# NVlabs/FoundationPose

Measured on NVIDIA H100. Metric: pose-hypotheses/sec at 640x480 RGB-D, 252 hyp, 5 refine iters, higher is better.
Workload: dtype f16

## Files before the change

### foundationpose_b200/csrc/fp_api_ops.cu

```cuda
#include "../../include/fpose.h"
#include "fp_common.cuh"
#include "fp_attn.cuh"
#include "fp_crop.cuh"
#include "fp_gemm.cuh"

#include <vector>

namespace fp {
const char* get_last_error();
int prof_collect(int kind, double* total_ms, double* total_work, int* launches);
int pose_errors_launch(const float* pts, int P, const float* pred, int N, const float* gt, int n_gt, float* add_out,
                       float* adds_out, cudaStream_t stream);
}

static int check_device_ptr(const void* p, const char* what) {
  int dev = 0;
  FP_CUDA_OK(cudaGetDevice(&dev));
  cudaPointerAttributes a;
  const cudaError_t e = cudaPointerGetAttributes(&a, p);
  if (e != cudaSuccess) {
    cudaGetLastError();
    fp::set_last_error("fp_pose_errors: %s: cudaPointerGetAttributes failed (%s)", what, cudaGetErrorString(e));
    return -1;
  }
// ... 97 lines not shown
  ap.k_off = 512;
  ap.v_off = 1024;
  ap.group_col_stride = 0;
  ap.n_groups = 1;
  ap.out = reinterpret_cast<__half*>(out);
  ap.ld_out = 512;
  ap.out_group_stride = 0;
  ap.B = B;
  ap.T = 400;
  ap.n_heads = 4;
  ap.scale = 0.08838834764831845f;
  cudaStream_t st = reinterpret_cast<cudaStream_t>(stream);
  (void)impl;
  return fp::attn_tc_launch(ap, st);
}

static fp::GemmLayer to_gemm_layer(const fp_gemm_layer_t* l) {
  fp::GemmLayer L;
  L.kind = l->kind;
  L.n_img = l->n_img;
  L.Hin = l->Hin;
  L.Win = l->Win;
  L.Cin = l->Cin;
  L.Cout = l->Cout;
  L.in = l->in;
  L.w = l->w;
  L.bias = l->bias;
  L.res = l->res;
  L.res_ld = l->res_ld;
  L.out = l->out;
  L.out_ld = l->out_ld;
  L.out_split = l->out_split;
  L.post_add = l->post_add;
  L.relu = l->relu;
  return L;
}

int fp_op_gemm_layer(const fp_gemm_layer_t* l, void* stream) {
  if (!l) {
    fp::set_last_error("fp_op_gemm_layer: null layer");
    return -1;
  }
  return fp::gemm_layer_launch(to_gemm_layer(l), reinterpret_cast<cudaStream_t>(stream));
}

int fp_op_gemm_tile_n(const fp_gemm_layer_t* l, int* tile_n) {
  if (!l || !tile_n) {
    fp::set_last_error("fp_op_gemm_tile_n: null argument");
    return -1;
  }
  return fp::gemm_layer_tile_n(to_gemm_layer(l), tile_n);
}

int fp_pose_errors(const float* pts, int P, const float* pred, int N, const float* gt, int n_gt, float* add_out,
                   float* adds_out, void* stream) {
  FP_REQUIRE(P >= 1 && P <= FP_METRICS_MAX_POINTS, "fp_pose_errors: P = %d outside [1, %d]", P, FP_METRICS_MAX_POINTS);
  FP_REQUIRE(N >= 0 && N <= FP_METRICS_MAX_POSES, "fp_pose_errors: N = %d outside [0, %d]", N, FP_METRICS_MAX_POSES);
  FP_REQUIRE(n_gt == 1 || n_gt == N, "fp_pose_errors: n_gt = %d, must be 1 or N = %d", n_gt, N);
  if (N == 0) return 0;
  FP_REQUIRE(pts && pred && gt, "fp_pose_errors: null input pointer");
  const void* ptrs[5] = {pts, pred, gt, add_out, adds_out};
  const char* names[5] = {"pts", "pred", "gt", "add_out", "adds_out"};
  for (int i = 0; i < 5; ++i)
    if (ptrs[i] && check_device_ptr(ptrs[i], names[i])) return -1;
  return fp::pose_errors_launch(pts, P, pred, N, gt, n_gt, add_out, adds_out, reinterpret_cast<cudaStream_t>(stream));
}

}
```

### foundationpose_b200/csrc/fp_common.cuh

```cuda
#pragma once
#include <cuda.h>
#include <cuda_fp16.h>
#include <cuda_runtime.h>
#include <stdint.h>
#include <stdio.h>
#include <string.h>

#include <atomic>

namespace fp {

void note_launches(int n);
unsigned long long launch_count();
void set_capturing(bool on);
inline bool device_bit_test(const std::atomic<unsigned long long>& m) {
  int d = 0;
  cudaGetDevice(&d);
  return (m.load(std::memory_order_acquire) >> (d & 63)) & 1ull;
}
inline void device_bit_set(std::atomic<unsigned long long>& m) {
  int d = 0;
  cudaGetDevice(&d);
  m.fetch_or(1ull << (d & 63), std::memory_order_release);
}
// ... 104 lines not shown
  asm volatile("cp.async.bulk.tensor.5d.global.shared::cta.bulk_group [%0, {%2, %3, %4, %5, %6}], [%1];" ::"l"(
                   reinterpret_cast<uint64_t>(map)),
               "r"(smem_u32(src)), "r"(c0), "r"(c1), "r"(c2), "r"(c3), "r"(c4)
               : "memory");
}
__device__ __forceinline__ void tma_prefetch_desc(const CUtensorMap* map) {
  asm volatile("prefetch.tensormap [%0];" ::"l"(reinterpret_cast<uint64_t>(map)) : "memory");
}

__device__ __forceinline__ uint32_t cluster_nctarank() {
  uint32_t r;
  asm volatile("mov.u32 %0, %%cluster_nctarank;" : "=r"(r));
  return r;
}
__device__ __forceinline__ uint32_t cluster_ctarank() {
  uint32_t r;
  asm volatile("mov.u32 %0, %%cluster_ctarank;" : "=r"(r));
  return r;
}
__device__ __forceinline__ void cluster_sync_all() {
  asm volatile("barrier.cluster.arrive.release.aligned;" ::: "memory");
  asm volatile("barrier.cluster.wait.acquire.aligned;" ::: "memory");
}

template <uint32_t N>
__device__ __forceinline__ void regs_release() {
  asm volatile("setmaxnreg.dec.sync.aligned.u32 %0;" ::"n"(N));
}
template <uint32_t N>
__device__ __forceinline__ void regs_acquire() {
  asm volatile("setmaxnreg.inc.sync.aligned.u32 %0;" ::"n"(N));
}

__device__ __forceinline__ void wgmma_fence() { asm volatile("wgmma.fence.sync.aligned;" ::: "memory"); }
__device__ __forceinline__ void wgmma_commit() { asm volatile("wgmma.commit_group.sync.aligned;" ::: "memory"); }
template <int N>
__device__ __forceinline__ void wgmma_wait() {
  asm volatile("wgmma.wait_group.sync.aligned %0;" ::"n"(N) : "memory");
}
template <int N>
__device__ __forceinline__ void fence_regs(float (&d)[N]) {
#pragma unroll
  for (int i = 0; i < N; ++i) asm volatile("" : "+f"(d[i])::"memory");
}

__device__ __forceinline__ uint64_t gmma_desc_sw128(uint32_t smem_addr, uint32_t sbo = 1024) {
  uint64_t d = 0;
  d |= (uint64_t)((smem_addr & 0x3FFFF) >> 4);
  d |= (uint64_t)1 << 16;
  d |= (uint64_t)(sbo >> 4) << 32;
  d |= (uint64_t)1 << 62;
  return d;
}
__device__ __forceinline__ uint64_t gmma_desc_mn_sw128(uint32_t smem_addr, uint32_t lbo) {
  uint64_t d = 0;
  d |= (uint64_t)((smem_addr & 0x3FFFF) >> 4);
  d |= (uint64_t)((lbo >> 4) & 0x3FFF) << 16;
  d |= (uint64_t)(1024 >> 4) << 32;
  d |= (uint64_t)1 << 62;
  return d;
}
__device__ __forceinline__ uint64_t gmma_desc_linear(uint32_t smem_addr, uint32_t lbo, uint32_t sbo) {
  uint64_t d = 0;
  d |= (uint64_t)((smem_addr & 0x3FFFF) >> 4);
  d |= (uint64_t)(lbo >> 4) << 16;
  d |= (uint64_t)(sbo >> 4) << 32;
  return d;
}

__device__ __forceinline__ uint32_t pack_half2(float a, float b) {
  __half2 h = __floats2half2_rn(a, b);
  return *reinterpret_cast<uint32_t*>(&h);
}

}
```

### foundationpose_b200/csrc/fp_gemm.cu

```cuda
#include "fp_gemm.cuh"

#include <stdarg.h>
#include <stdlib.h>
#include <string.h>

#include <mutex>
#include <vector>

#include "fp_common.cuh"
#include "fp_wgmma.cuh"

namespace fp {

static std::atomic<unsigned long long> g_launch_count{0};
static thread_local bool t_capturing = false;
void note_launches(int n) {
  if (!t_capturing) g_launch_count.fetch_add((unsigned long long)n, std::memory_order_relaxed);
}
unsigned long long launch_count() { return g_launch_count.load(std::memory_order_relaxed); }
void set_capturing(bool on) { t_capturing = on; }

std::atomic<bool> g_prof_on{false};
static std::mutex g_prof_mu;

// ... 49 lines not shown

static thread_local char t_last_error[1024] = "";
void set_last_error(const char* fmt, ...) {
  va_list ap;
  va_start(ap, fmt);
  vsnprintf(t_last_error, sizeof(t_last_error), fmt, ap);
  va_end(ap);
}
const char* get_last_error() { return t_last_error; }

static thread_local int t_pdl_skip = 0;
void pdl_skip_next() { t_pdl_skip = 1; }

bool pdl_enabled() {
  if (t_pdl_skip) {
    t_pdl_skip = 0;
    return false;
  }
  static int on = -1;
  if (on < 0) {
    const char* e = getenv("FPOSE_PDL");
    on = (e && e[0] == '0') ? 0 : 1;
  }
  return on != 0;
}

struct GemmParams {
  int lg_bw, lg_bh;
  int bw, bh, bn;
  int tiles_w, tiles_h, tiles_n, n_tiles_n, total_tiles;
  int num_kb, chunks_per_tap;
  int dim_w, dim_h, dim_n;
  short tap_off[9][5];
  int Ho, Wo, n_img, Cout;
  const float* bias;
  int has_res;
  int odim_h, odim_n;
  int out_split;
  const float* post_add;
  int relu;
  double alg_flops;
};

constexpr int kBlockM = 128;
constexpr int kBlockK = 64;
constexpr int kABytes = kBlockM * kBlockK * 2;
constexpr int kTileThreads = 384;
constexpr int kSlabBytes = kBlockM * 64 * 2;
constexpr int kSmemOptIn = 232448;

constexpr int kWideSlabs = 2;
constexpr int kWideProducerRegs = 40;
constexpr int kWideConsumerRegs = 232;
template <int BN>
struct TileCfg {
  static constexpr int kBBytes = BN * kBlockK * 2;
  static constexpr int kStageBytes = kABytes + kBBytes;
  static constexpr int kBatches = BN / 64;
  static constexpr bool kAlternate = BN > 128;
  static constexpr int kSlabs = kAlternate ? kWideSlabs : kBatches;
  static constexpr int kStagingBytes = kSlabs * kSlabBytes;
  static constexpr int kRing = kSmemOptIn - kStagingBytes - 1024  - 256 ;
  static constexpr int kStages = (kRing / kStageBytes) > 8 ? 8 : (kRing / kStageBytes);
  static constexpr int kSmemBytes = kStages * kStageBytes + kStagingBytes + 1024 + 256;
  static_assert(kSmemBytes <= kSmemOptIn, "tile configuration exceeds the 227 KB opt-in shared memory");
  static_assert((2 * kStages + kSlabs) * 8 <= 256, "the mbarriers must fit their 256 bytes");
  static_assert(kBatches % kSlabs == 0, "every slab must take the same number of batches per tile");
};

template <int BN>
__global__ void __launch_bounds__(kTileThreads, 1)
    gemm_tile_kernel(const __grid_constant__ CUtensorMap map_a, const __grid_constant__ CUtensorMap map_b,
                     const __grid_constant__ CUtensorMap map_out, const __grid_constant__ CUtensorMap map_res,
                     const __grid_constant__ GemmParams p) {
  using Cfg = TileCfg<BN>;
  constexpr int S = Cfg::kStages;
  constexpr int NSLAB = Cfg::kSlabs;
  constexpr int NB = Cfg::kBatches;
  constexpr bool kAlt = Cfg::kAlternate;
  extern __shared__ uint8_t smem_raw[];
  uint8_t* smem = smem_raw + ((1024u - (smem_u32(smem_raw) & 1023u)) & 1023u);
  uint8_t* staging = smem + S * Cfg::kStageBytes;
  uint64_t* bars = reinterpret_cast<uint64_t*>(staging + Cfg::kStagingBytes);
  uint64_t* full = bars;
  uint64_t* empty = bars + S;
  uint64_t* res_full = bars + 2 * S;

  const int m_tiles = p.tiles_w * p.tiles_h * p.tiles_n;
  const int total = m_tiles * p.n_tiles_n;

  if (threadIdx.x == 0) {
    tma_prefetch_desc(&map_a);
    tma_prefetch_desc(&map_b);
    tma_prefetch_desc(&map_out);
    if (p.has_res) tma_prefetch_desc(&map_res);
    for (int s = 0; s < S; ++s) {
      mbar_init(&full[s], 1);
      mbar_init(&empty[s], 256);
    }
    for (int s = 0; s < (kAlt ? NSLAB : 1); ++s) mbar_init(&res_full[s], 1);
    mbar_fence_init();
  }
  __syncthreads();
  pdl_trigger();
  pdl_wait();

  auto decode = [&](int t, int& n_tile, int& tw, int& th, int& tn) {
    n_tile = t % p.n_tiles_n;
    const int m_tile = t / p.n_tiles_n;
    tw = m_tile % p.tiles_w;
    th = (m_tile / p.tiles_w) % p.tiles_h;
    tn = m_tile / (p.tiles_w * p.tiles_h);
  };

  if (threadIdx.x < 128) {
    if constexpr (BN > 128) regs_release<kWideProducerRegs>();
    if (threadIdx.x == 0) {
      int stage = 0, phase = 0;
      for (int t = blockIdx.x; t < total; t += gridDim.x) {
        int n_tile, tw, th, tn;
        decode(t, n_tile, tw, th, tn);
        int base[5] = {0, 0, 0, 0, 0};
        base[p.dim_w] += tw * p.bw;
        if (p.dim_h >= 0) base[p.dim_h] += th * p.bh;
        if (p.dim_n >= 0) base[p.dim_n] += tn * p.bn;
        int tap = 0, chunk = 0;
        for (int kb = 0; kb < p.num_kb; ++kb) {
          mbar_wait(&empty[stage], phase ^ 1);
          uint8_t* sa = smem + stage * Cfg::kStageBytes;
          mbar_expect_tx(&full[stage], Cfg::kStageBytes);
          tma_load_5d(&map_a, &full[stage], sa, base[0] + p.tap_off[tap][0] + chunk * kBlockK, base[1] + p.tap_off[tap][1],
                      base[2] + p.tap_off[tap][2], base[3] + p.tap_off[tap][3], base[4] + p.tap_off[tap][4]);
          tma_load_2d(&map_b, &full[stage], sa + kABytes, kb * kBlockK, n_tile * BN);
          if (++chunk == p.chunks_per_tap) {
            chunk = 0;
            ++tap;
          }
          if (++stage == S) {
            stage = 0;
            phase ^= 1;
          }
        }
      }
    }
    return;
  }

  if constexpr (BN > 128) regs_acquire<kWideConsumerRegs>();
  const int ct = threadIdx.x - 128;
  const int cw = ct >> 7;
  const int lane = threadIdx.x & 31;
  const int r0 = 64 * cw + 16 * ((ct >> 5) & 3) + (lane >> 2);
  const int cq = 2 * (lane & 3);
  const bool leader = (ct == 0);
  float acc[BN / 2];
#pragma unroll
  for (int i = 0; i < BN / 2; ++i) acc[i] = 0.f;
  int stage = 0, phase = 0, it = 0;
  for (int t = blockIdx.x; t < total; t += gridDim.x, ++it) {
    int n_tile, tw, th, tn;
    decode(t, n_tile, tw, th, tn);
    const int n0 = tn * p.bn;
    int n_o0 = n0, coff = 0;
    if (p.out_split > 0) {
      n_o0 = n0 % p.out_split;
      coff = (n0 / p.out_split) * p.Cout;
    }
    int oc[5] = {0, 0, 0, 0, 0}, rc[5] = {0, 0, 0, 0, 0};
    oc[1] = rc[1] = tw * p.bw;
    if (p.odim_h >= 0) oc[p.odim_h] = rc[p.odim_h] = th * p.bh;
    if (p.odim_n >= 0) {
      oc[p.odim_n] = n_o0;
      rc[p.odim_n] = n0;
    }
    if (leader) asm volatile("cp.async.bulk.wait_group.read 0;" ::: "memory");
    asm volatile("bar.sync 1, 256;" ::: "memory");
    if (leader && p.has_res) {
      for (int s = 0; s < NSLAB; ++s) {
        uint64_t* rb = &res_full[kAlt ? s : 0];
        if (kAlt || s == 0) mbar_expect_tx(rb, kAlt ? kSlabBytes : NSLAB * kSlabBytes);
        tma_load_5d(&map_res, rb, staging + s * kSlabBytes, n_tile * BN + s * 64, rc[1], rc[2], rc[3], rc[4]);
      }
    }

    int prev = -1;
    for (int kb = 0; kb < p.num_kb; ++kb) {
      mbar_wait(&full[stage], phase);
      const uint32_t sa = smem_u32(smem + stage * Cfg::kStageBytes);
      const uint64_t da = gmma_desc_sw128(sa + (uint32_t)cw * 8192u);
      const uint64_t db = gmma_desc_sw128(sa + kABytes);
      wgmma_fence();
#pragma unroll
      for (int k = 0; k < kBlockK / 16; ++k)
        Wgmma<BN>::ss(acc, da + (uint64_t)(2 * k), db + (uint64_t)(2 * k), (kb > 0 || k > 0) ? 1u : 0u);
      wgmma_commit();
      if (prev >= 0) {
        wgmma_wait<1>();
        mbar_arrive(&empty[prev]);
      }
      prev = stage;
      if (++stage == S) {
        stage = 0;
        phase ^= 1;
      }
    }
    const float* bias = p.bias + n_tile * BN;
    const float* pap[2] = {nullptr, nullptr};
    if (p.post_add) {
#pragma unroll
      for (int h = 0; h < 2; ++h) {
        const int row = r0 + 8 * h;
        const int jj = row & (p.bw - 1), ii = (row >> p.lg_bw) & (p.bh - 1);
        const int i = th * p.bh + ii, j = min(tw * p.bw + jj, p.Wo - 1);
        pap[h] = p.post_add + (size_t)(i * p.Wo + j) * p.Cout + n_tile * BN;
      }
    }
    float2 pe[8][2];
    auto load_pe = [&](int b) {
#pragma unroll
      for (int jl = 0; jl < 8; ++jl)
#pragma unroll
        for (int h = 0; h < 2; ++h) pe[jl][h] = __ldg(reinterpret_cast<const float2*>(pap[h] + 64 * b + 8 * jl + cq));
    };
    if (p.post_add) load_pe(0);
    wgmma_wait<0>();
    fence_regs(acc);
    if (prev >= 0) mbar_arrive(&empty[prev]);

#pragma unroll
    for (int b = 0; b < NB; ++b) {
      const int s = kAlt ? (b & 1) : b;
      uint8_t* slab = staging + s * kSlabBytes;
      if (kAlt && p.has_res && b > 0 && b + 1 < NB) {
        if (leader) {
          asm volatile("cp.async.bulk.wait_group.read 0;" ::: "memory");
          uint64_t* rb = &res_full[(b + 1) & 1];
          mbar_expect_tx(rb, kSlabBytes);
          tma_load_5d(&map_res, rb, staging + ((b + 1) & 1) * kSlabBytes, n_tile * BN + (b + 1) * 64, rc[1], rc[2],
                      rc[3], rc[4]);
        }
      }
      if (p.has_res && (kAlt || b == 0))
        mbar_wait(&res_full[kAlt ? s : 0], (uint32_t)((it * (NB / NSLAB) + b / NSLAB) & 1));
#pragma unroll
      for (int jh = 0; jh < 8; jh += 4) {
        float2 bb[4];
        __half2 rv[4][2];
#pragma unroll
        for (int jl = 0; jl < 4; ++jl) {
          bb[jl] = __ldg(reinterpret_cast<const float2*>(bias + 64 * b + 8 * (jh + jl) + cq));
          if (p.has_res) {
#pragma unroll
            for (int h = 0; h < 2; ++h) {
              const int row = r0 + 8 * h;
              rv[jl][h] = *reinterpret_cast<const __half2*>(slab + row * 128 + (((uint32_t)(jh + jl) ^ (uint32_t)(row & 7)) << 4) + cq * 2);
            }
          }
        }
#pragma unroll
        for (int jl = 0; jl < 4; ++jl) {
          const int j = 8 * b + jh + jl;
#pragma unroll
          for (int h = 0; h < 2; ++h) {
            const int row = r0 + 8 * h;
            uint32_t* cell = reinterpret_cast<uint32_t*>(slab + row * 128 + (((uint32_t)(jh + jl) ^ (uint32_t)(row & 7)) << 4) + cq * 2);
            float a0 = acc[4 * j + 2 * h] + bb[jl].x, a1 = acc[4 * j + 2 * h + 1] + bb[jl].y;
            if (p.has_res) {
              const float2 r = __half22float2(rv[jl][h]);
              a0 += r.x;
              a1 += r.y;
            }
            if (p.relu) {
              a0 = fmaxf(a0, 0.f);
              a1 = fmaxf(a1, 0.f);
            }
            if (p.post_add) {
              a0 += pe[jh + jl][h].x;
              a1 += pe[jh + jl][h].y;
            }
            *cell = pack_half2(a0, a1);
          }
        }
      }
      if (p.post_add && b + 1 < NB) load_pe(b + 1);
      if (kAlt || b == NB - 1) {
        asm volatile("fence.proxy.async.shared::cta;" ::: "memory");
        if (kAlt && leader) asm volatile("cp.async.bulk.wait_group.read 0;" ::: "memory");
        asm volatile("bar.sync 1, 256;" ::: "memory");
        if (leader) {
          for (int q = kAlt ? s : 0; q < (kAlt ? s + 1 : NSLAB); ++q)
            tma_store_5d(&map_out, staging + q * kSlabBytes, coff + n_tile * BN + (kAlt ? 64 * b : 64 * q), oc[1],
                         oc[2], oc[3], oc[4]);
          asm volatile("cp.async.bulk.commit_group;" ::: "memory");
        }
      }
    }
  }
  if (leader) asm volatile("cp.async.bulk.wait_group 0;" ::: "memory");
}

static int g_num_sms = 0;

typedef CUresult (*EncodeTiledFn)(CUtensorMap*, CUtensorMapDataType, cuuint32_t, void*, const cuuint64_t*,
                                  const cuuint64_t*, const cuuint32_t*, const cuuint32_t*,
                                  CUtensorMapInterleave, CUtensorMapSwizzle, CUtensorMapL2promotion,
                                  CUtensorMapFloatOOBfill);

static EncodeTiledFn get_encode_fn() {
  static EncodeTiledFn fn = nullptr;
  static std::once_flag once;
  std::call_once(once, [] {
    void* p = nullptr;
    cudaDriverEntryPointQueryResult qres;
    if (cudaGetDriverEntryPoint("cuTensorMapEncodeTiled", &p, cudaEnableDefault, &qres) == cudaSuccess &&
        qres == cudaDriverEntryPointSuccess)
      fn = reinterpret_cast<EncodeTiledFn>(p);
  });
  return fn;
}

static int encode_map(CUtensorMap* map, const void* base, int rank, const uint64_t* dims,
                      const uint64_t* strides_bytes , const uint32_t* box, bool swizzle128 = true) {
  EncodeTiledFn fn = get_encode_fn();
  FP_REQUIRE(fn != nullptr, "cuTensorMapEncodeTiled entry point not available (no CUDA driver?)");
  cuuint64_t gdim[5];
  cuuint64_t gstr[4];
  cuuint32_t bdim[5];
  cuuint32_t estr[5];
  for (int i = 0; i < rank; ++i) {
    gdim[i] = dims[i];
    bdim[i] = box[i];
    estr[i] = 1;
  }
  for (int i = 0; i < rank - 1; ++i) gstr[i] = strides_bytes[i];
  CUresult r = fn(map, CU_TENSOR_MAP_DATA_TYPE_FLOAT16, (cuuint32_t)rank, const_cast<void*>(base), gdim, gstr,
                  bdim, estr, CU_TENSOR_MAP_INTERLEAVE_NONE, swizzle128 ? CU_TENSOR_MAP_SWIZZLE_128B : CU_TENSOR_MAP_SWIZZLE_NONE,
                  CU_TENSOR_MAP_L2_PROMOTION_L2_256B, CU_TENSOR_MAP_FLOAT_OOB_FILL_NONE);
  FP_REQUIRE(r == CUDA_SUCCESS,
             "cuTensorMapEncodeTiled failed (%d): rank %d dims [%llu %llu %llu %llu %llu] box [%u %u %u %u %u]",
             (int)r, rank, (unsigned long long)dims[0], (unsigned long long)(rank > 1 ? dims[1] : 0),
             (unsigned long long)(rank > 2 ? dims[2] : 0), (unsigned long long)(rank > 3 ? dims[3] : 0),
             (unsigned long long)(rank > 4 ? dims[4] : 0), box[0], rank > 1 ? box[1] : 0, rank > 2 ? box[2] : 0,
             rank > 3 ? box[3] : 0, rank > 4 ? box[4] : 0);
  return 0;
}

int encode_map_f16(CUtensorMap* map, const void* base, int rank, const uint64_t* dims, const uint64_t* strides_bytes,
                   const uint32_t* box) {
  return encode_map(map, base, rank, dims, strides_bytes, box);
}
int encode_map_f16_linear(CUtensorMap* map, const void* base, int rank, const uint64_t* dims,
                          const uint64_t* strides_bytes, const uint32_t* box) {
  return encode_map(map, base, rank, dims, strides_bytes, box, false);
}
int num_sms() {
  if (g_num_sms == 0) {
    int dev = 0;
    if (cudaGetDevice(&dev) != cudaSuccess) return 0;
    if (cudaDeviceGetAttribute(&g_num_sms, cudaDevAttrMultiProcessorCount, dev) != cudaSuccess) return 0;
  }
  return g_num_sms;
}

static int ilog2(int v) {
  int l = 0;
  while ((1 << l) < v) ++l;
  return l;
}

template <int BN>
static int launch_bn(const CUtensorMap& ma, const CUtensorMap& mb, const CUtensorMap& mo, const CUtensorMap& mr,
                     const GemmParams& p, cudaStream_t stream) {
  using Cfg = TileCfg<BN>;
  static std::atomic<unsigned long long> attr_mask{0};
  if (!device_bit_test(attr_mask)) {
    FP_CUDA_OK(cudaFuncSetAttribute(gemm_tile_kernel<BN>, cudaFuncAttributeMaxDynamicSharedMemorySize, Cfg::kSmemBytes));
    device_bit_set(attr_mask);
  }
  const int sms = num_sms();
  FP_REQUIRE(sms > 0, "no CUDA device");
  const int grid = p.total_tiles < sms ? p.total_tiles : sms;
  prof_mark_begin(0, p.alg_flops, stream);
  FP_CUDA_OK(launch_pdl(gemm_tile_kernel<BN>, dim3(grid), dim3(kTileThreads), Cfg::kSmemBytes, stream, 1, ma, mb, mo, mr, p));
  prof_mark_end(stream);
  note_launches(1);
  FP_CUDA_OK(cudaGetLastError());
  return 0;
}

int stem_conv_launch(const GemmLayer& L, cudaStream_t stream);

static int gemm_layer_plan(const GemmLayer& L, cudaStream_t stream, int* tile_n) {
  if (L.kind == LK_CONV7_S2) {
    if (tile_n) {
      *tile_n = 64;
      return 0;
    }
    return stem_conv_launch(L, stream);
  }
  GemmParams p;
  memset(&p, 0, sizeof(p));
  CUtensorMap ma, mb;
  const uint64_t E = 2;
  int Ho, Wo, taps, ktot;
  int BN;
  uint64_t dims[5], str[4];
  uint32_t box[5];

  switch (L.kind) {
    case LK_LINEAR: {
      FP_REQUIRE(L.Cin % 64 == 0, "LINEAR: K=%d not a multiple of 64", L.Cin);
      Ho = 1;
      Wo = L.Win;
      taps = 1;
      p.chunks_per_tap = L.Cin / 64;
      p.bw = 128; p.bh = 1; p.bn = 1;
      p.dim_w = 1; p.dim_h = -1; p.dim_n = -1;
      dims[0] = L.Cin; dims[1] = L.Win; dims[2] = 1; dims[3] = 1; dims[4] = 1;
      str[0] = L.Cin * E; str[1] = str[0] * L.Win; str[2] = str[1]; str[3] = str[1];
      box[0] = 64; box[1] = 128; box[2] = 1; box[3] = 1; box[4] = 1;
      p.tiles_w = (L.Win + 127) / 128; p.tiles_h = 1; p.tiles_n = 1;
      break;
    }
    case LK_CONV3_S1: {
      FP_REQUIRE(L.Cin % 64 == 0, "CONV3_S1: Cin=%d not a multiple of 64", L.Cin);
      Ho = L.Hin; Wo = L.Win;
      taps = 9;
      p.chunks_per_tap = L.Cin / 64;
      if (Wo % 8 == 0 && Ho % 8 == 0) { p.bw = 8; p.bh = 8; p.bn = 2; }
      else if (Wo % 4 == 0 && Ho % 4 == 0) { p.bw = 4; p.bh = 4; p.bn = 8; }
      else FP_REQUIRE(false, "CONV3_S1: unsupported spatial size %dx%d", Ho, Wo);
      const uint64_t sw_ = (uint64_t)L.Cin * E, sh_ = sw_ * L.Win, sn_ = sh_ * L.Hin;
      p.dim_w = 1; p.dim_h = 2; p.dim_n = 3;
      dims[0] = L.Cin; dims[1] = L.Win; dims[2] = L.Hin; dims[3] = L.n_img; dims[4] = 1;
      str[0] = sw_; str[1] = sh_; str[2] = sn_; str[3] = sn_ * L.n_img;
      box[0] = 64; box[1] = p.bw; box[2] = p.bh; box[3] = p.bn; box[4] = 1;
      for (int r = 0; r < 3; ++r)
        for (int s = 0; s < 3; ++s) {
          p.tap_off[r * 3 + s][1] = (short)(s - 1);
          p.tap_off[r * 3 + s][2] = (short)(r - 1);
        }
      p.tiles_w = Wo / p.bw; p.tiles_h = Ho / p.bh; p.tiles_n = (L.n_img + p.bn - 1) / p.bn;
      break;
    }
    case LK_CONV3_S2: {
// ... 5 lines not shown
      if (Wo % 8 == 0 && Ho % 8 == 0) { p.bw = 8; p.bh = 8; p.bn = 2; }
      else if (Wo % 4 == 0 && Ho % 4 == 0) { p.bw = 4; p.bh = 4; p.bn = 8; }
      else FP_REQUIRE(false, "CONV3_S2: unsupported output size %dx%d", Ho, Wo);
      p.dim_w = 1; p.dim_h = 3; p.dim_n = 4;
      dims[0] = 2 * L.Cin; dims[1] = Wo; dims[2] = 2; dims[3] = Ho; dims[4] = L.n_img;
      str[0] = 2 * L.Cin * E; str[1] = (uint64_t)L.Win * L.Cin * E; str[2] = 2 * str[1];
      str[3] = (uint64_t)L.Hin * L.Win * L.Cin * E;
      box[0] = 64; box[1] = p.bw; box[2] = 1; box[3] = p.bh; box[4] = p.bn;
      for (int r = 0; r < 3; ++r)
        for (int s = 0; s < 3; ++s) {
          const int t = r * 3 + s;
          p.tap_off[t][0] = (short)((s == 1 ? 0 : 1) * L.Cin);
          p.tap_off[t][1] = (short)(s == 0 ? -1 : 0);
          p.tap_off[t][2] = (short)(r == 1 ? 0 : 1);
          p.tap_off[t][3] = (short)(r == 0 ? -1 : 0);
        }
      p.tiles_w = Wo / p.bw; p.tiles_h = Ho / p.bh; p.tiles_n = (L.n_img + p.bn - 1) / p.bn;
      break;
    }
    default:
      FP_REQUIRE(false, "unknown layer kind %d", L.kind);
  }
  ktot = taps * L.Cin;
  p.num_kb = ktot / 64;
  p.lg_bw = ilog2(p.bw);
  p.lg_bh = ilog2(p.bh);

  constexpr int kWideMinWaves = 8;
  constexpr int kWideMinKBlocks = 16;
  const int m_tiles = p.tiles_w * p.tiles_h * p.tiles_n;
  if (L.Cout % 256 == 0 && p.num_kb >= kWideMinKBlocks) {
    const int sms = num_sms();
    FP_REQUIRE(sms > 0, "no CUDA device");
    BN = (long long)m_tiles * (L.Cout / 256) >= (long long)kWideMinWaves * sms ? 256 : 128;
  } else if (L.Cout % 128 == 0) BN = 128;
  else if (L.Cout % 64 == 0) BN = 64;
  else FP_REQUIRE(false, "Cout=%d must be a multiple of 64", L.Cout);
  p.n_tiles_n = L.Cout / BN;
  p.total_tiles = p.tiles_w * p.tiles_h * p.tiles_n * p.n_tiles_n;
  p.Ho = Ho; p.Wo = Wo; p.n_img = L.n_img; p.Cout = L.Cout;
  p.bias = L.bias;
  p.has_res = L.res != nullptr;
  p.out_split = L.out_split;
  p.post_add = L.post_add;
  p.relu = L.relu;
  {
    const double k_real = (double)taps * L.Cin;
    p.alg_flops = 2.0 * (double)L.n_img * Ho * Wo * L.Cout * k_real;
  }
  FP_REQUIRE(L.out_ld % 8 == 0 && (!L.res || L.res_ld % 8 == 0), "out_ld / res_ld must be multiples of 8");
  FP_REQUIRE(L.out_split == 0 || L.out_split % p.bn == 0,
             "out_split=%d must be a multiple of the tile's image count %d (pad the A/B batch boundary)", L.out_split,
             p.bn);
  if (tile_n) {
    *tile_n = BN;
    return 0;
  }
  if (p.total_tiles == 0) return 0;

  int rc = encode_map(&ma, L.in, 5, dims, str, box);
  if (rc) return rc;
  uint64_t wd[2] = {(uint64_t)ktot, (uint64_t)L.Cout};
  uint64_t ws[1] = {(uint64_t)ktot * E};
  uint32_t wb[2] = {64, (uint32_t)BN};
  rc = encode_map(&mb, L.w, 2, wd, ws, wb);
  if (rc) return rc;
  CUtensorMap mo, mr;
  {
    uint64_t od[5], os[4];
    uint32_t ob[5];
    const bool lin = (L.kind == LK_LINEAR);
    const int n_out = L.out_split > 0 ? (L.n_img - L.out_split) : L.n_img;
    FP_REQUIRE(n_out > 0, "out_split=%d leaves no output images (n_img=%d)", L.out_split, L.n_img);
    auto fill = [&](int ld, int nimg) {
      const uint64_t sw_ = (uint64_t)ld * E, sh_ = sw_ * Wo, sn_ = sh_ * Ho;
      od[0] = (uint64_t)ld;
      ob[0] = 64;
      od[4] = 1;
      ob[4] = 1;
      if (lin) {
        od[1] = (uint64_t)Wo; od[2] = 1; od[3] = 1;
        os[0] = sw_; os[1] = sh_; os[2] = sh_; os[3] = sh_;
        ob[1] = (uint32_t)p.bw; ob[2] = 1; ob[3] = 1;
      } else {
        od[1] = (uint64_t)Wo; od[2] = (uint64_t)Ho; od[3] = (uint64_t)nimg;
        os[0] = sw_; os[1] = sh_; os[2] = sn_; os[3] = sn_ * nimg;
        ob[1] = (uint32_t)p.bw; ob[2] = (uint32_t)p.bh; ob[3] = (uint32_t)p.bn;
      }
    };
    p.odim_h = lin ? -1 : 2;
    p.odim_n = lin ? -1 : 3;
    fill(L.out_ld, n_out);
    rc = encode_map(&mo, L.out, 5, od, os, ob);
    if (rc) return rc;
    if (L.res) {
      fill(L.res_ld, L.n_img);
      rc = encode_map(&mr, L.res, 5, od, os, ob);
      if (rc) return rc;
    } else {
      mr = mo;
    }
  }
  if (BN == 256) return launch_bn<256>(ma, mb, mo, mr, p, stream);
  return BN == 128 ? launch_bn<128>(ma, mb, mo, mr, p, stream) : launch_bn<64>(ma, mb, mo, mr, p, stream);
}

int gemm_layer_launch(const GemmLayer& L, cudaStream_t stream) { return gemm_layer_plan(L, stream, nullptr); }

int gemm_layer_tile_n(const GemmLayer& L, int* tile_n) { return gemm_layer_plan(L, nullptr, tile_n); }

}
```

### foundationpose_b200/csrc/fp_gemm.cuh

```cuda
#pragma once
#include <cuda.h>
#include <cuda_runtime.h>
#include <stdint.h>

#include <atomic>

namespace fp {

enum LayerKind : int {
  LK_LINEAR = 0,
  LK_CONV3_S1 = 1,
  LK_CONV3_S2 = 2,
  LK_CONV7_S2 = 3,
};

struct GemmLayer {
  int kind;
  int n_img;
  int Hin, Win;
  int Cin;
  int Cout;
  const void* in;
  const void* w;
  const float* bias;
  const void* res;
  int res_ld;
  void* out;
  int out_ld;
  int out_split;
  const float* post_add;
  int relu;
};

int gemm_layer_launch(const GemmLayer& L, cudaStream_t stream);
int gemm_layer_tile_n(const GemmLayer& L, int* tile_n);


void prof_mark_begin(int kind, double work, cudaStream_t stream);
void prof_mark_end(cudaStream_t stream);
extern std::atomic<bool> g_prof_on;

}
```

### foundationpose_b200/ops.py

```python
import ctypes as C

import torch

from . import _lib
from ._lib import lib


def _ptr(t):
    return None if t is None else C.c_void_p(t.data_ptr())


def _stream():
    return C.c_void_p(torch.cuda.current_stream().cuda_stream)


def _require_cuda(*ts):
    for t in ts:
        if t is not None and not t.is_cuda:
            raise _lib.FposeError("libfpose operators need CUDA tensors (there is no CPU path)")


def gemm_layer(kind, x, w_packed, bias, *, n_img, Hin, Win, Cin, Cout, out=None, out_ld=None, out_split=0,
               res=None, res_ld=0, post_add=None, relu=False):
    _require_cuda(x, w_packed, bias, res, post_add, out)
    assert x.dtype == torch.float16 and w_packed.dtype == torch.float16 and bias.dtype == torch.float32
    if kind == _lib.LAYER_LINEAR:
        Ho, Wo = 1, Win
    elif kind == _lib.LAYER_CONV3_S1:
        Ho, Wo = Hin, Win
    else:
        Ho, Wo = Hin // 2, Win // 2
    if out is None:
        out_ld = Cout
        out = torch.empty(n_img, Ho, Wo, Cout, dtype=torch.float16, device=x.device)
    L = _lib.GemmLayer(kind, n_img, Hin, Win, Cin, Cout, _ptr(x), _ptr(w_packed), _ptr(bias), _ptr(res),
                       res_ld, _ptr(out), out_ld, out_split, _ptr(post_add), 1 if relu else 0)
    _lib.check(lib.fp_op_gemm_layer(C.byref(L), _stream()), "fp_op_gemm_layer")
    return out


def gemm_tile_n(kind, *, n_img, Hin, Win, Cin, Cout, out_split=0):
    lib.fp_op_gemm_tile_n.argtypes = [C.POINTER(_lib.GemmLayer), C.POINTER(C.c_int)]
    lib.fp_op_gemm_tile_n.restype = C.c_int
    L = _lib.GemmLayer(kind, n_img, Hin, Win, Cin, Cout, None, None, None, None, 0, None, Cout, out_split, None, 0)
    tile_n = C.c_int(0)
    _lib.check(lib.fp_op_gemm_tile_n(C.byref(L), C.byref(tile_n)), "fp_op_gemm_tile_n")
    return tile_n.value


lib.fp_op_attention.argtypes = [C.c_void_p, C.c_void_p, C.c_int, C.c_int, C.c_void_p]
lib.fp_op_attention.restype = C.c_int


def attention(qkv, impl=1):
    _require_cuda(qkv)
    assert qkv.dtype == torch.float16 and qkv.shape[1] == 1536 and qkv.shape[0] % 400 == 0
    B = qkv.shape[0] // 400
    out = torch.empty(qkv.shape[0], 512, dtype=torch.float16, device=qkv.device)
    _lib.check(lib.fp_op_attention(_ptr(qkv), _ptr(out), B, impl, _stream()), "fp_op_attention")
    return out
```

### include/fpose.h

```cpp
#ifndef FPOSE_H_
#define FPOSE_H_

#include <stddef.h>
#include <stdint.h>

#ifdef __cplusplus
extern "C" {
#endif

const char* fp_last_error(void);
unsigned long long fp_launch_count(void);

int fp_prof_enable(int on);
int fp_prof_collect(int kind, double* total_ms, double* total_work, int* launches);


#define FP_LAYER_LINEAR 0
#define FP_LAYER_CONV3_S1 1
#define FP_LAYER_CONV3_S2 2
#define FP_LAYER_CONV7_S2 3

typedef struct fp_gemm_layer {
  int kind;
  int n_img;
  int Hin, Win;
  int Cin;
  int Cout;
  const void* in;
  const void* w;
  const float* bias;
  const void* res;
  int res_ld;
  void* out;
  int out_ld;
  int out_split;
  const float* post_add;
  int relu;
} fp_gemm_layer_t;

int fp_op_gemm_layer(const fp_gemm_layer_t* layer, void* stream);
int fp_op_gemm_tile_n(const fp_gemm_layer_t* layer, int* tile_n);

int fp_op_attention(const void* qkv, void* out, int B, int impl, void* stream);



#define FP_METRICS_MAX_POINTS 131072
#define FP_METRICS_MAX_POSES (1 << 24)
int fp_pose_errors(const float* pts, int P, const float* pred, int N, const float* gt, int n_gt,
                   float* add_out, float* adds_out, void* stream);

typedef struct fp_ctx fp_ctx;

int fp_create(fp_ctx** ctx);
int fp_destroy(fp_ctx* ctx);

int fp_set_config(fp_ctx* ctx, int which, float crop_ratio, float rot_normalizer);

typedef struct fp_tensor {
  const char* name;
  const void* data;
  int dtype;
  long long numel;
} fp_tensor_t;

int fp_load_network(fp_ctx* ctx, int which, const fp_tensor_t* tensors, int n);

int fp_set_mesh(fp_ctx* ctx, int V, int F, const float* pos, const float* nrm, const float* uv, const float* vcol,
                const int* faces, const unsigned char* tex_rgb, int Ht, int Wt, float diameter);
#define FP_MAX_MESHES 64
int fp_set_mesh_slot(fp_ctx* ctx, int slot, int V, int F, const float* pos, const float* nrm, const float* uv,
                     const float* vcol, const int* faces, const unsigned char* tex_rgb, int Ht, int Wt, float diameter);
int fp_mesh_info(fp_ctx* ctx, int* info);

#define FP_FRAME_ON_DEVICE 1
#define FP_FRAME_FILTER_DEPTH 2
int fp_set_frame(fp_ctx* ctx, const unsigned char* rgb, const float* depth, const float* K, int H, int W, int flags,
                 float zfar, void* stream);
int fp_set_xyz_map(fp_ctx* ctx, const float* xyz, void* stream);
int fp_get_depth(fp_ctx* ctx, float* depth_out_dev, float* xyz_out_dev, void* stream);

int fp_start_poses(fp_ctx* ctx, const unsigned char* mask, int mask_on_device, const float* rot_grid, int N,
                   float* poses_out, float* info_out, void* stream);

int fp_make_crops(fp_ctx* ctx, const float* poses, int N, int mode, void* crops_out, float* dbg_out, float* win_out,
                  void* stream);
int fp_set_crop_tile(fp_ctx* ctx, int tile);
int fp_crop_stats(fp_ctx* ctx, const float* poses, int N, int mode, int* stats_out_host, void* stream);

int fp_refine(fp_ctx* ctx, const float* poses_in, int N, int iterations, float* poses_out, float* last_trans,
              float* last_rot, void* stream);

int fp_score(fp_ctx* ctx, const float* poses, int N, float* scores_out, int* best_out, void* stream);
int fp_score_features(fp_ctx* ctx, const float* poses, int N, float* feats_out, void* stream);
// ... 59 lines not shown
```

Measured before the change: 3604.

## Load halo patch once per 3x3 conv tile and reuse across all nine taps

For stride-1 3x3 convolutions with 8-wide tiles and the 128-wide N tile, the producer now loads one (bw+2)x(bh+2) input halo patch per channel chunk into a dedicated 4-slot patch ring. The wgmma A descriptors then address each tap as an offset into that patch, so the 9 per-tap A loads are replaced by one load and the ring holds only weights. The epilogue is split per warpgroup with named barriers, and one warpgroup is started a few stages later via a skew mbarrier. This gives up some ring depth and adds more synchronisation in exchange for much less A-operand TMA traffic. The existing per-tap path stays available through a tap_boxes switch.

```diff
diff --git a/foundationpose_b200/csrc/fp_api_ops.cu b/foundationpose_b200/csrc/fp_api_ops.cu
--- a/foundationpose_b200/csrc/fp_api_ops.cu
+++ b/foundationpose_b200/csrc/fp_api_ops.cu
@@ -173,6 +173,23 @@
   return fp::gemm_layer_tile_n(to_gemm_layer(l), tile_n);
 }
 
+int fp_op_gemm_patch(const fp_gemm_layer_t* l, int* patch) {
+  if (!l || !patch) {
+    fp::set_last_error("fp_op_gemm_patch: null argument");
+    return -1;
+  }
+  int tile_n = 0;
+  return fp::gemm_layer_tile_n(to_gemm_layer(l), &tile_n, patch);
+}
+
+int fp_op_gemm_layer_mode(const fp_gemm_layer_t* l, int tap_boxes, int* patched, void* stream) {
+  if (!l) {
+    fp::set_last_error("fp_op_gemm_layer_mode: null layer");
+    return -1;
+  }
+  return fp::gemm_layer_launch(to_gemm_layer(l), reinterpret_cast<cudaStream_t>(stream), tap_boxes != 0, patched);
+}
+
 int fp_pose_errors(const float* pts, int P, const float* pred, int N, const float* gt, int n_gt, float* add_out,
                    float* adds_out, void* stream) {
   FP_REQUIRE(P >= 1 && P <= FP_METRICS_MAX_POINTS, "fp_pose_errors: P = %d outside [1, %d]", P, FP_METRICS_MAX_POINTS);
diff --git a/foundationpose_b200/csrc/fp_common.cuh b/foundationpose_b200/csrc/fp_common.cuh
--- a/foundationpose_b200/csrc/fp_common.cuh
+++ b/foundationpose_b200/csrc/fp_common.cuh
@@ -180,6 +180,9 @@
   d |= (uint64_t)1 << 62;
   return d;
 }
+__device__ __forceinline__ uint64_t gmma_desc_sw128_patch(uint32_t slot_addr, int w, int r, int s) {
+  return gmma_desc_sw128(slot_addr + (uint32_t)(100 * w + 10 * r + s) * 128u, 1280);
+}
 __device__ __forceinline__ uint64_t gmma_desc_mn_sw128(uint32_t smem_addr, uint32_t lbo) {
   uint64_t d = 0;
   d |= (uint64_t)((smem_addr & 0x3FFFF) >> 4);
diff --git a/foundationpose_b200/csrc/fp_gemm.cu b/foundationpose_b200/csrc/fp_gemm.cu
--- a/foundationpose_b200/csrc/fp_gemm.cu
+++ b/foundationpose_b200/csrc/fp_gemm.cu
@@ -125,39 +125,52 @@
 constexpr int kWideSlabs = 2;
 constexpr int kWideProducerRegs = 40;
 constexpr int kWideConsumerRegs = 232;
-template <int BN>
+
+constexpr int kPatchBytes = 64 * 10 * 10 * 2 * 2;
+constexpr int kPatchSlots = 4;
+template <int BN, bool PATCH = false>
 struct TileCfg {
   static constexpr int kBBytes = BN * kBlockK * 2;
-  static constexpr int kStageBytes = kABytes + kBBytes;
+  static constexpr int kPatchRegion = PATCH ? kPatchSlots * kPatchBytes : 0;
+  static constexpr int kStageBytes = (PATCH ? 0 : kABytes) + kBBytes;
   static constexpr int kBatches = BN / 64;
   static constexpr bool kAlternate = BN > 128;
   static constexpr int kSlabs = kAlternate ? kWideSlabs : kBatches;
   static constexpr int kStagingBytes = kSlabs * kSlabBytes;
-  static constexpr int kRing = kSmemOptIn - kStagingBytes - 1024  - 256 ;
+  static constexpr int kRing = kSmemOptIn - kPatchRegion - kStagingBytes - 1024  - 256 ;
   static constexpr int kStages = (kRing / kStageBytes) > 8 ? 8 : (kRing / kStageBytes);
-  static constexpr int kSmemBytes = kStages * kStageBytes + kStagingBytes + 1024 + 256;
+  static constexpr int kSmemBytes = kPatchRegion + kStages * kStageBytes + kStagingBytes + 1024 + 256;
   static_assert(kSmemBytes <= kSmemOptIn, "tile configuration exceeds the 227 KB opt-in shared memory");
-  static_assert((2 * kStages + kSlabs) * 8 <= 256, "the mbarriers must fit their 256 bytes");
+  static_assert((2 * kStages + kSlabs + (PATCH ? 2 * kPatchSlots + 1 : 0)) * 8 <= 256,
+                "the mbarriers must fit their 256 bytes");
+  static_assert(!PATCH || kSlabs >= 2, "the split epilogue keeps one residual mbarrier per warpgroup in res_full");
   static_assert(kBatches % kSlabs == 0, "every slab must take the same number of batches per tile");
+  static_assert(!PATCH || BN == 128, "patch mode is built for the 128-wide tile only");
+  static_assert(!PATCH || kStages == 5, "BN = 128 patch plan: 4 patch slots, 2 slabs, 5 weight stages");
 };
 
-template <int BN>
+template <int BN, bool PATCH>
 __global__ void __launch_bounds__(kTileThreads, 1)
     gemm_tile_kernel(const __grid_constant__ CUtensorMap map_a, const __grid_constant__ CUtensorMap map_b,
                      const __grid_constant__ CUtensorMap map_out, const __grid_constant__ CUtensorMap map_res,
                      const __grid_constant__ GemmParams p) {
-  using Cfg = TileCfg<BN>;
+  using Cfg = TileCfg<BN, PATCH>;
   constexpr int S = Cfg::kStages;
   constexpr int NSLAB = Cfg::kSlabs;
   constexpr int NB = Cfg::kBatches;
   constexpr bool kAlt = Cfg::kAlternate;
   extern __shared__ uint8_t smem_raw[];
   uint8_t* smem = smem_raw + ((1024u - (smem_u32(smem_raw) & 1023u)) & 1023u);
-  uint8_t* staging = smem + S * Cfg::kStageBytes;
+  uint8_t* patches = smem;
+  uint8_t* ring = smem + Cfg::kPatchRegion;
+  uint8_t* staging = ring + S * Cfg::kStageBytes;
   uint64_t* bars = reinterpret_cast<uint64_t*>(staging + Cfg::kStagingBytes);
   uint64_t* full = bars;
   uint64_t* empty = bars + S;
   uint64_t* res_full = bars + 2 * S;
+  uint64_t* patch_full = bars + 2 * S + NSLAB;
+  uint64_t* patch_empty = bars + 2 * S + NSLAB + kPatchSlots;
+  uint64_t* skew = bars + 2 * S + NSLAB + 2 * kPatchSlots;
 
   const int m_tiles = p.tiles_w * p.tiles_h * p.tiles_n;
   const int total = m_tiles * p.n_tiles_n;
@@ -171,7 +184,14 @@
       mbar_init(&full[s], 1);
       mbar_init(&empty[s], 256);
     }
-    for (int s = 0; s < (kAlt ? NSLAB : 1); ++s) mbar_init(&res_full[s], 1);
+    for (int s = 0; s < (kAlt || PATCH ? NSLAB : 1); ++s) mbar_init(&res_full[s], 1);
+    if constexpr (PATCH) {
+      for (int s = 0; s < kPatchSlots; ++s) {
+        mbar_init(&patch_full[s], 1);
+        mbar_init(&patch_empty[s], 256);
+      }
+      mbar_init(skew, 1);
+    }
     mbar_fence_init();
   }
   __syncthreads();
@@ -190,6 +210,7 @@
     if constexpr (BN > 128) regs_release<kWideProducerRegs>();
     if (threadIdx.x == 0) {
       int stage = 0, phase = 0;
+      int pg = 0;
       for (int t = blockIdx.x; t < total; t += gridDim.x) {
         int n_tile, tw, th, tn;
         decode(t, n_tile, tw, th, tn);
@@ -199,12 +220,25 @@
         if (p.dim_n >= 0) base[p.dim_n] += tn * p.bn;
         int tap = 0, chunk = 0;
         for (int kb = 0; kb < p.num_kb; ++kb) {
+          if constexpr (PATCH) {
+            if (tap == 0) {
+              const int ps = pg % kPatchSlots;
+              mbar_wait(&patch_empty[ps], ((pg / kPatchSlots) & 1) ^ 1);
+              mbar_expect_tx(&patch_full[ps], kPatchBytes);
+              tma_load_5d(&map_a, &patch_full[ps], patches + ps * kPatchBytes, base[0] + p.tap_off[0][0] + chunk * kBlockK,
+                          base[1] + p.tap_off[0][1], base[2] + p.tap_off[0][2], base[3] + p.tap_off[0][3],
+                          base[4] + p.tap_off[0][4]);
+              ++pg;
+            }
+          }
           mbar_wait(&empty[stage], phase ^ 1);
-          uint8_t* sa = smem + stage * Cfg::kStageBytes;
+          uint8_t* sa = ring + stage * Cfg::kStageBytes;
           mbar_expect_tx(&full[stage], Cfg::kStageBytes);
-          tma_load_5d(&map_a, &full[stage], sa, base[0] + p.tap_off[tap][0] + chunk * kBlockK, base[1] + p.tap_off[tap][1],
-                      base[2] + p.tap_off[tap][2], base[3] + p.tap_off[tap][3], base[4] + p.tap_off[tap][4]);
-          tma_load_2d(&map_b, &full[stage], sa + kABytes, kb * kBlockK, n_tile * BN);
+          if constexpr (!PATCH)
+            tma_load_5d(&map_a, &full[stage], sa, base[0] + p.tap_off[tap][0] + chunk * kBlockK,
+                        base[1] + p.tap_off[tap][1], base[2] + p.tap_off[tap][2], base[3] + p.tap_off[tap][3],
+                        base[4] + p.tap_off[tap][4]);
+          tma_load_2d(&map_b, &full[stage], sa + (PATCH ? 0 : kABytes), kb * kBlockK, n_tile * BN);
           if (++chunk == p.chunks_per_tap) {
             chunk = 0;
             ++tap;
@@ -225,11 +259,19 @@
   const int lane = threadIdx.x & 31;
   const int r0 = 64 * cw + 16 * ((ct >> 5) & 3) + (lane >> 2);
   const int cq = 2 * (lane & 3);
-  const bool leader = (ct == 0);
+  constexpr bool kSplit = PATCH;
+  constexpr int kSkew = S - 1;
+  const bool leader = kSplit ? ((ct & 127) == 0) : (ct == 0);
+  const uint32_t wg_bytes = kSplit ? (uint32_t)cw * (kSlabBytes / 2) : 0u;
+  auto epi_sync = [&]() {
+    if constexpr (kSplit) asm volatile("bar.sync %0, 128;" ::"r"(2 + cw) : "memory");
+    else asm volatile("bar.sync 1, 256;" ::: "memory");
+  };
   float acc[BN / 2];
 #pragma unroll
   for (int i = 0; i < BN / 2; ++i) acc[i] = 0.f;
   int stage = 0, phase = 0, it = 0;
+  if (kSplit && cw == 1 && blockIdx.x < total) mbar_wait(skew, 0);
   for (int t = blockIdx.x; t < total; t += gridDim.x, ++it) {
     int n_tile, tw, th, tn;
     decode(t, n_tile, tw, th, tn);
@@ -243,38 +285,56 @@
     oc[1] = rc[1] = tw * p.bw;
     if (p.odim_h >= 0) oc[p.odim_h] = rc[p.odim_h] = th * p.bh;
     if (p.odim_n >= 0) {
-      oc[p.odim_n] = n_o0;
-      rc[p.odim_n] = n0;
+      oc[p.odim_n] = n_o0 + (kSplit ? cw : 0);
+      rc[p.odim_n] = n0 + (kSplit ? cw : 0);
     }
     if (leader) asm volatile("cp.async.bulk.wait_group.read 0;" ::: "memory");
-    asm volatile("bar.sync 1, 256;" ::: "memory");
+    epi_sync();
     if (leader && p.has_res) {
       for (int s = 0; s < NSLAB; ++s) {
-        uint64_t* rb = &res_full[kAlt ? s : 0];
-        if (kAlt || s == 0) mbar_expect_tx(rb, kAlt ? kSlabBytes : NSLAB * kSlabBytes);
-        tma_load_5d(&map_res, rb, staging + s * kSlabBytes, n_tile * BN + s * 64, rc[1], rc[2], rc[3], rc[4]);
-      }
-    }
-
-    int prev = -1;
+        uint64_t* rb = &res_full[kSplit ? cw : (kAlt ? s : 0)];
+        if (kAlt || s == 0) mbar_expect_tx(rb, kAlt ? kSlabBytes : NSLAB * (kSlabBytes >> (kSplit ? 1 : 0)));
+        tma_load_5d(&map_res, rb, staging + s * kSlabBytes + wg_bytes, n_tile * BN + s * 64, rc[1], rc[2], rc[3],
+                    rc[4]);
+      }
+    }
+
+    int prev = -1, prev_patch = -1;
+    const int pg0 = it * p.chunks_per_tap;
+    int tap = 0, chunk = 0;
     for (int kb = 0; kb < p.num_kb; ++kb) {
+      uint64_t da;
+      int ps = 0;
+      if constexpr (PATCH) {
+        ps = (pg0 + chunk) % kPatchSlots;
+        if (tap == 0) mbar_wait(&patch_full[ps], (uint32_t)(((pg0 + chunk) / kPatchSlots) & 1));
+        const int r = tap / 3;
+        da = gmma_desc_sw128_patch(smem_u32(patches + ps * kPatchBytes), cw, r, tap - 3 * r);
+      }
       mbar_wait(&full[stage], phase);
-      const uint32_t sa = smem_u32(smem + stage * Cfg::kStageBytes);
-      const uint64_t da = gmma_desc_sw128(sa + (uint32_t)cw * 8192u);
-      const uint64_t db = gmma_desc_sw128(sa + kABytes);
+      const uint32_t sa = smem_u32(ring + stage * Cfg::kStageBytes);
+      if constexpr (!PATCH) da = gmma_desc_sw128(sa + (uint32_t)cw * 8192u);
+      const uint64_t db = gmma_desc_sw128(sa + (PATCH ? 0 : kABytes));
       wgmma_fence();
 #pragma unroll
       for (int k = 0; k < kBlockK / 16; ++k)
         Wgmma<BN>::ss(acc, da + (uint64_t)(2 * k), db + (uint64_t)(2 * k), (kb > 0 || k > 0) ? 1u : 0u);
       wgmma_commit();
+      if (kSplit && ct == 0 && it == 0 && kb == min(kSkew, p.num_kb) - 1) mbar_arrive(skew);
       if (prev >= 0) {
         wgmma_wait<1>();
         mbar_arrive(&empty[prev]);
+        if (PATCH && prev_patch >= 0) mbar_arrive(&patch_empty[prev_patch]);
       }
       prev = stage;
+      prev_patch = (PATCH && tap == 8) ? ps : -1;
       if (++stage == S) {
         stage = 0;
         phase ^= 1;
+      }
+      if (++chunk == p.chunks_per_tap) {
+        chunk = 0;
+        ++tap;
       }
     }
     const float* bias = p.bias + n_tile * BN;
@@ -299,6 +359,7 @@
     wgmma_wait<0>();
     fence_regs(acc);
     if (prev >= 0) mbar_arrive(&empty[prev]);
+    if (PATCH && prev_patch >= 0) mbar_arrive(&patch_empty[prev_patch]);
 
 #pragma unroll
     for (int b = 0; b < NB; ++b) {
@@ -314,7 +375,7 @@
         }
       }
       if (p.has_res && (kAlt || b == 0))
-        mbar_wait(&res_full[kAlt ? s : 0], (uint32_t)((it * (NB / NSLAB) + b / NSLAB) & 1));
+        mbar_wait(&res_full[kSplit ? cw : (kAlt ? s : 0)], (uint32_t)((it * (NB / NSLAB) + b / NSLAB) & 1));
 #pragma unroll
       for (int jh = 0; jh < 8; jh += 4) {
         float2 bb[4];
@@ -359,11 +420,11 @@
       if (kAlt || b == NB - 1) {
         asm volatile("fence.proxy.async.shared::cta;" ::: "memory");
         if (kAlt && leader) asm volatile("cp.async.bulk.wait_group.read 0;" ::: "memory");
-        asm volatile("bar.sync 1, 256;" ::: "memory");
+        epi_sync();
         if (leader) {
           for (int q = kAlt ? s : 0; q < (kAlt ? s + 1 : NSLAB); ++q)
-            tma_store_5d(&map_out, staging + q * kSlabBytes, coff + n_tile * BN + (kAlt ? 64 * b : 64 * q), oc[1],
-                         oc[2], oc[3], oc[4]);
+            tma_store_5d(&map_out, staging + q * kSlabBytes + wg_bytes, coff + n_tile * BN + (kAlt ? 64 * b : 64 * q),
+                         oc[1], oc[2], oc[3], oc[4]);
           asm volatile("cp.async.bulk.commit_group;" ::: "memory");
         }
       }
@@ -441,20 +502,21 @@
   return l;
 }
 
-template <int BN>
+template <int BN, bool PATCH = false>
 static int launch_bn(const CUtensorMap& ma, const CUtensorMap& mb, const CUtensorMap& mo, const CUtensorMap& mr,
                      const GemmParams& p, cudaStream_t stream) {
-  using Cfg = TileCfg<BN>;
+  using Cfg = TileCfg<BN, PATCH>;
   static std::atomic<unsigned long long> attr_mask{0};
   if (!device_bit_test(attr_mask)) {
-    FP_CUDA_OK(cudaFuncSetAttribute(gemm_tile_kernel<BN>, cudaFuncAttributeMaxDynamicSharedMemorySize, Cfg::kSmemBytes));
+    FP_CUDA_OK(cudaFuncSetAttribute(gemm_tile_kernel<BN, PATCH>, cudaFuncAttributeMaxDynamicSharedMemorySize,
+                                    Cfg::kSmemBytes));
     device_bit_set(attr_mask);
   }
   const int sms = num_sms();
   FP_REQUIRE(sms > 0, "no CUDA device");
   const int grid = p.total_tiles < sms ? p.total_tiles : sms;
   prof_mark_begin(0, p.alg_flops, stream);
-  FP_CUDA_OK(launch_pdl(gemm_tile_kernel<BN>, dim3(grid), dim3(kTileThreads), Cfg::kSmemBytes, stream, 1, ma, mb, mo, mr, p));
+  FP_CUDA_OK(launch_pdl(gemm_tile_kernel<BN, PATCH>, dim3(grid), dim3(kTileThreads), Cfg::kSmemBytes, stream, 1, ma, mb, mo, mr, p));
   prof_mark_end(stream);
   note_launches(1);
   FP_CUDA_OK(cudaGetLastError());
@@ -463,7 +525,8 @@
 
 int stem_conv_launch(const GemmLayer& L, cudaStream_t stream);
 
-static int gemm_layer_plan(const GemmLayer& L, cudaStream_t stream, int* tile_n) {
+static int gemm_layer_plan(const GemmLayer& L, cudaStream_t stream, bool tap_boxes, int* tile_n, int* patch) {
+  if (patch) *patch = 0;
   if (L.kind == LK_CONV7_S2) {
     if (tile_n) {
       *tile_n = 64;
@@ -575,6 +638,13 @@
   FP_REQUIRE(L.out_split == 0 || L.out_split % p.bn == 0,
              "out_split=%d must be a multiple of the tile's image count %d (pad the A/B batch boundary)", L.out_split,
              p.bn);
+  const bool use_patch =
+      !tap_boxes && L.kind == LK_CONV3_S1 && p.bw == 8 && p.chunks_per_tap <= kPatchSlots && BN == 128;
+  if (use_patch) {
+    box[1] = p.bw + 2;
+    box[2] = p.bh + 2;
+  }
+  if (patch) *patch = use_patch ? 1 : 0;
   if (tile_n) {
     *tile_n = BN;
     return 0;
@@ -608,7 +678,7 @@
       } else {
         od[1] = (uint64_t)Wo; od[2] = (uint64_t)Ho; od[3] = (uint64_t)nimg;
         os[0] = sw_; os[1] = sh_; os[2] = sn_; os[3] = sn_ * nimg;
-        ob[1] = (uint32_t)p.bw; ob[2] = (uint32_t)p.bh; ob[3] = (uint32_t)p.bn;
+        ob[1] = (uint32_t)p.bw; ob[2] = (uint32_t)p.bh; ob[3] = use_patch ? 1u : (uint32_t)p.bn;
       }
     };
     p.odim_h = lin ? -1 : 2;
@@ -624,12 +694,17 @@
       mr = mo;
     }
   }
+  if (use_patch) return launch_bn<128, true>(ma, mb, mo, mr, p, stream);
   if (BN == 256) return launch_bn<256>(ma, mb, mo, mr, p, stream);
   return BN == 128 ? launch_bn<128>(ma, mb, mo, mr, p, stream) : launch_bn<64>(ma, mb, mo, mr, p, stream);
 }
 
-int gemm_layer_launch(const GemmLayer& L, cudaStream_t stream) { return gemm_layer_plan(L, stream, nullptr); }
-
-int gemm_layer_tile_n(const GemmLayer& L, int* tile_n) { return gemm_layer_plan(L, nullptr, tile_n); }
-
-}
+int gemm_layer_launch(const GemmLayer& L, cudaStream_t stream, bool tap_boxes, int* patched) {
+  return gemm_layer_plan(L, stream, tap_boxes, nullptr, patched);
+}
+
+int gemm_layer_tile_n(const GemmLayer& L, int* tile_n, int* patch) {
+  return gemm_layer_plan(L, nullptr, false, tile_n, patch);
+}
+
+}
diff --git a/foundationpose_b200/csrc/fp_gemm.cuh b/foundationpose_b200/csrc/fp_gemm.cuh
--- a/foundationpose_b200/csrc/fp_gemm.cuh
+++ b/foundationpose_b200/csrc/fp_gemm.cuh
@@ -32,8 +32,8 @@
   int relu;
 };
 
-int gemm_layer_launch(const GemmLayer& L, cudaStream_t stream);
-int gemm_layer_tile_n(const GemmLayer& L, int* tile_n);
+int gemm_layer_launch(const GemmLayer& L, cudaStream_t stream, bool tap_boxes = false, int* patched = nullptr);
+int gemm_layer_tile_n(const GemmLayer& L, int* tile_n, int* patch = nullptr);
 
 
 void prof_mark_begin(int kind, double work, cudaStream_t stream);
diff --git a/foundationpose_b200/ops.py b/foundationpose_b200/ops.py
--- a/foundationpose_b200/ops.py
+++ b/foundationpose_b200/ops.py
@@ -22,6 +22,26 @@
 
 def gemm_layer(kind, x, w_packed, bias, *, n_img, Hin, Win, Cin, Cout, out=None, out_ld=None, out_split=0,
                res=None, res_ld=0, post_add=None, relu=False):
+    L, out = _gemm_args(kind, x, w_packed, bias, n_img, Hin, Win, Cin, Cout, out, out_ld, out_split, res, res_ld,
+                        post_add, relu)
+    _lib.check(lib.fp_op_gemm_layer(C.byref(L), _stream()), "fp_op_gemm_layer")
+    return out
+
+
+def gemm_layer_mode(kind, x, w_packed, bias, *, tap_boxes, n_img, Hin, Win, Cin, Cout, out=None, out_ld=None,
+                    out_split=0, res=None, res_ld=0, post_add=None, relu=False):
+    lib.fp_op_gemm_layer_mode.argtypes = [C.POINTER(_lib.GemmLayer), C.c_int, C.POINTER(C.c_int), C.c_void_p]
+    lib.fp_op_gemm_layer_mode.restype = C.c_int
+    L, out = _gemm_args(kind, x, w_packed, bias, n_img, Hin, Win, Cin, Cout, out, out_ld, out_split, res, res_ld,
+                        post_add, relu)
+    patched = C.c_int(-1)
+    _lib.check(lib.fp_op_gemm_layer_mode(C.byref(L), 1 if tap_boxes else 0, C.byref(patched), _stream()),
+               "fp_op_gemm_layer_mode")
+    return out, bool(patched.value)
+
+
+def _gemm_args(kind, x, w_packed, bias, n_img, Hin, Win, Cin, Cout, out, out_ld, out_split, res, res_ld, post_add,
+               relu):
     _require_cuda(x, w_packed, bias, res, post_add, out)
     assert x.dtype == torch.float16 and w_packed.dtype == torch.float16 and bias.dtype == torch.float32
     if kind == _lib.LAYER_LINEAR:
@@ -35,8 +55,7 @@
         out = torch.empty(n_img, Ho, Wo, Cout, dtype=torch.float16, device=x.device)
     L = _lib.GemmLayer(kind, n_img, Hin, Win, Cin, Cout, _ptr(x), _ptr(w_packed), _ptr(bias), _ptr(res),
                        res_ld, _ptr(out), out_ld, out_split, _ptr(post_add), 1 if relu else 0)
-    _lib.check(lib.fp_op_gemm_layer(C.byref(L), _stream()), "fp_op_gemm_layer")
-    return out
+    return L, out
 
 
 def gemm_tile_n(kind, *, n_img, Hin, Win, Cin, Cout, out_split=0):
@@ -46,6 +65,15 @@
     tile_n = C.c_int(0)
     _lib.check(lib.fp_op_gemm_tile_n(C.byref(L), C.byref(tile_n)), "fp_op_gemm_tile_n")
     return tile_n.value
+
+
+def gemm_patch(kind, *, n_img, Hin, Win, Cin, Cout, out_split=0):
+    lib.fp_op_gemm_patch.argtypes = [C.POINTER(_lib.GemmLayer), C.POINTER(C.c_int)]
+    lib.fp_op_gemm_patch.restype = C.c_int
+    L = _lib.GemmLayer(kind, n_img, Hin, Win, Cin, Cout, None, None, None, None, 0, None, Cout, out_split, None, 0)
+    patch = C.c_int(0)
+    _lib.check(lib.fp_op_gemm_patch(C.byref(L), C.byref(patch)), "fp_op_gemm_patch")
+    return bool(patch.value)
 
 
 lib.fp_op_attention.argtypes = [C.c_void_p, C.c_void_p, C.c_int, C.c_int, C.c_void_p]
diff --git a/include/fpose.h b/include/fpose.h
--- a/include/fpose.h
+++ b/include/fpose.h
@@ -40,6 +40,8 @@
 
 int fp_op_gemm_layer(const fp_gemm_layer_t* layer, void* stream);
 int fp_op_gemm_tile_n(const fp_gemm_layer_t* layer, int* tile_n);
+int fp_op_gemm_patch(const fp_gemm_layer_t* layer, int* patch);
+int fp_op_gemm_layer_mode(const fp_gemm_layer_t* layer, int tap_boxes, int* patched, void* stream);
 
 int fp_op_attention(const void* qkv, void* out, int B, int impl, void* stream);
 
```

Result: faster. 3644, median of 6 (+1.1%).
